# HITRainer/EAVSR

Measured on NVIDIA B200. Metric: LR frames/s, EAVSR+ x4, 270x480, higher is better.
Workload: dtype bf16

## Files before the change

### eavsr_b200/csrc/align_fused.cu

```cuda
#include "common.cuh"

namespace eavsr {
namespace {

constexpr int MX_TH = 8, MX_TW = 16;
constexpr int MX_IH = MX_TH + 4, MX_IW = MX_TW + 4;
constexpr int MX_YH = MX_TH + 2, MX_YW = MX_TW + 2;
constexpr int MX_C = 64;
constexpr int MX_THREADS = 256;

__device__ __forceinline__ void lds8(const __nv_bfloat16* p, float* f) {
  const uint4 u = *reinterpret_cast<const uint4*>(p);
  f[0] = bf16lo_to_f32(u.x); f[1] = bf16hi_to_f32(u.x); f[2] = bf16lo_to_f32(u.y); f[3] = bf16hi_to_f32(u.y);
  f[4] = bf16lo_to_f32(u.z); f[5] = bf16hi_to_f32(u.z); f[6] = bf16lo_to_f32(u.w); f[7] = bf16hi_to_f32(u.w);
}
__device__ __forceinline__ void lds8(const float* p, float* f) {
  const float4 a = *reinterpret_cast<const float4*>(p), b = *reinterpret_cast<const float4*>(p + 4);
  f[0] = a.x; f[1] = a.y; f[2] = a.z; f[3] = a.w; f[4] = b.x; f[5] = b.y; f[6] = b.z; f[7] = b.w;
}

template <typename T> struct MixSmem {
  T in[MX_IH * MX_IW][MX_C];
  T y[MX_YH * MX_YW][MX_C];
  float w1[9][MX_C];
// ... 7 lines not shown
adapt_mix_kernel(const T* __restrict__ a, const T* __restrict__ b, const T* __restrict__ w1g,
                 const T* __restrict__ b1g, const T* __restrict__ w2g, const T* __restrict__ b2g,
                 T* __restrict__ out, int H, int W, float slope) {
  extern __shared__ __align__(16) uint8_t mix_smem_raw[];
  MixSmem<T>& S = *reinterpret_cast<MixSmem<T>*>(mix_smem_raw);
  constexpr int VEC = 16 / sizeof(T);
  constexpr int CPP = MX_C / VEC;
  const int half = blockIdx.z & 1, n = blockIdx.z >> 1;
  const int y0 = blockIdx.y * MX_TH, x0 = blockIdx.x * MX_TW;
  const T* src = (half ? b : a) + (size_t)n * H * W * MX_C;
  const int tid = threadIdx.x;

  for (int i = tid; i < 9 * MX_C; i += MX_THREADS) {
    const int tap = i / MX_C, c = i % MX_C;
    S.w1[tap][c] = to_f32<T>(w1g[(size_t)(half * MX_C + c) * 9 + tap]);
    S.w2[tap][c] = to_f32<T>(w2g[((size_t)(half * (MX_C / 2) + (c >> 1)) * 2 + (c & 1)) * 9 + tap]);
  }
  for (int i = tid; i < MX_C; i += MX_THREADS) S.b1[i] = to_f32<T>(b1g[half * MX_C + i]);
  for (int i = tid; i < MX_C / 2; i += MX_THREADS) S.b2[i] = to_f32<T>(b2g[half * (MX_C / 2) + i]);

  for (int i = tid; i < MX_IH * MX_IW * CPP; i += MX_THREADS) {
    const int p = i / CPP, ch = i % CPP;
    const int gy = y0 - 2 + p / MX_IW, gx = x0 - 2 + p % MX_IW;
    const bool ok = gy >= 0 && gy < H && gx >= 0 && gx < W;
    const T* g = ok ? src + ((size_t)gy * W + gx) * MX_C + ch * VEC : src;
    const int sz = ok ? 16 : 0;
    asm volatile("cp.async.cg.shared.global [%0], [%1], 16, %2;\n" ::"r"(smem_u32(&S.in[p][ch * VEC])), "l"(g), "r"(sz));
  }
  cp_async_commit();
  cp_async_wait<0>();
  __syncthreads();

  const int c0 = (tid & 7) * 8;
  float wr[9][8], br[8];
#pragma unroll
  for (int tap = 0; tap < 9; ++tap)
#pragma unroll
    for (int e = 0; e < 8; ++e) wr[tap][e] = S.w1[tap][c0 + e];
#pragma unroll
  for (int e = 0; e < 8; ++e) br[e] = S.b1[c0 + e];

  auto st8 = [](T* p, const float* f) {
    if constexpr (sizeof(T) == 2) {
      VecLoad<T, 8>::st(p, f);
    } else {
      *reinterpret_cast<float4*>(p) = make_float4(f[0], f[1], f[2], f[3]);
      *reinterpret_cast<float4*>(p + 4) = make_float4(f[4], f[5], f[6], f[7]);
    }
  };
  static_assert(MX_YW % 2 == 0 && MX_TW % 2 == 0, "pixel pairs");
  for (int i = tid; i < MX_YH * (MX_YW / 2) * (MX_C / 8); i += MX_THREADS) {
    const int pp = i / (MX_C / 8);
    const int yy = pp / (MX_YW / 2), xx = (pp % (MX_YW / 2)) * 2;
    float acc[2][8];
#pragma unroll
    for (int e = 0; e < 8; ++e) acc[0][e] = acc[1][e] = br[e];
#pragma unroll
    for (int r = 0; r < 3; ++r) {
      float v[4][8];
#pragma unroll
      for (int c = 0; c < 4; ++c) lds8(&S.in[(yy + r) * MX_IW + xx + c][c0], v[c]);
#pragma unroll
      for (int t = 0; t < 3; ++t)
#pragma unroll
        for (int e = 0; e < 8; ++e) {
          acc[0][e] += wr[r * 3 + t][e] * v[t][e];
          acc[1][e] += wr[r * 3 + t][e] * v[t + 1][e];
        }
    }
    const int gy = y0 - 1 + yy;
#pragma unroll
    for (int k = 0; k < 2; ++k) {
      const int gx = x0 - 1 + xx + k;
      const bool inside = gy >= 0 && gy < H && gx >= 0 && gx < W;
      float o[8];
#pragma unroll
      for (int e = 0; e < 8; ++e) {
        const float v = acc[k][e] > 0.f ? acc[k][e] : acc[k][e] * slope;
        o[e] = inside ? v : 0.f;
      }
      st8(&S.y[yy * MX_YW + xx + k][c0], o);
    }
  }
  __syncthreads();

#pragma unroll
  for (int tap = 0; tap < 9; ++tap)
#pragma unroll
    for (int e = 0; e < 8; ++e) wr[tap][e] = S.w2[tap][c0 + e];
  for (int i = tid; i < MX_TH * (MX_TW / 2) * (MX_C / 8); i += MX_THREADS) {
    const int pp = i / (MX_C / 8);
    const int yy = pp / (MX_TW / 2), xx = (pp % (MX_TW / 2)) * 2;
    const int gy = y0 + yy, gx = x0 + xx;
    if (gy >= H || gx >= W) continue;
    float acc[2][4];
#pragma unroll
    for (int e = 0; e < 4; ++e) acc[0][e] = acc[1][e] = S.b2[(c0 >> 1) + e];
#pragma unroll
    for (int r = 0; r < 3; ++r) {
      float v[4][8];
#pragma unroll
      for (int c = 0; c < 4; ++c) lds8(&S.y[(yy + r) * MX_YW + xx + c][c0], v[c]);
#pragma unroll
      for (int t = 0; t < 3; ++t)
#pragma unroll
        for (int e = 0; e < 8; ++e) {
          acc[0][e >> 1] += wr[r * 3 + t][e] * v[t][e];
          acc[1][e >> 1] += wr[r * 3 + t][e] * v[t + 1][e];
        }
    }
#pragma unroll
    for (int k = 0; k < 2; ++k) {
      if (gx + k >= W) continue;
      T* op = out + ((size_t)n * H * W + (size_t)gy * W + gx + k) * MX_C + half * (MX_C / 2) + (c0 >> 1);
      float o[4];
#pragma unroll
      for (int e = 0; e < 4; ++e) o[e] = acc[k][e] > 0.f ? acc[k][e] : acc[k][e] * slope;
      if constexpr (sizeof(T) == 2) {
        *reinterpret_cast<uint2*>(op) = make_uint2(pack_bf16x2(o[0], o[1]), pack_bf16x2(o[2], o[3]));
      } else {
        *reinterpret_cast<float4*>(op) = make_float4(o[0], o[1], o[2], o[3]);
      }
    }
  }
}

template <typename T>
__global__ void __launch_bounds__(256)
affine_offsets_kernel(const T* __restrict__ tm, Strides4 ts, const T* __restrict__ tr, Strides4 rs,
                      const T* __restrict__ ml, Strides4 ms, const T* __restrict__ tm_bias,
                      const T* __restrict__ tr_bias, const T* __restrict__ ml_bias, float* __restrict__ offset,
                      float* __restrict__ mask, int N, int D, int H, int W) {
  const long long idx = (long long)blockIdx.x * blockDim.x + threadIdx.x;
  const long long HW = (long long)H * W;
  if (idx >= (long long)N * D * HW) return;
  const int pix = (int)(idx % HW);
  const int g = (int)((idx / HW) % D);
  const int n = (int)(idx / (HW * D));
  const int y = pix / W, x = pix % W;
  const T* tp = tm + n * ts.n + y * ts.h + x * ts.w + (long long)(g * 4) * ts.c;
  const T* rp = tr + n * rs.n + y * rs.h + x * rs.w + (long long)(g * 2) * rs.c;
  float a = to_f32<T>(tp[0]), b = to_f32<T>(tp[ts.c]), c = to_f32<T>(tp[2 * ts.c]), d = to_f32<T>(tp[3 * ts.c]);
  float t0 = to_f32<T>(rp[0]), t1 = to_f32<T>(rp[rs.c]);
  if (tm_bias) {
    a += to_f32<T>(tm_bias[g * 4]); b += to_f32<T>(tm_bias[g * 4 + 1]);
    c += to_f32<T>(tm_bias[g * 4 + 2]); d += to_f32<T>(tm_bias[g * 4 + 3]);
  }
  if (tr_bias) { t0 += to_f32<T>(tr_bias[g * 2]); t1 += to_f32<T>(tr_bias[g * 2 + 1]); }
  float* op = offset + ((size_t)(n * D + g) * 18) * HW + pix;
#pragma unroll
  for (int k = 0; k < 9; ++k) {
    const float r0 = (float)(k / 3 - 1), r1 = (float)(k % 3 - 1);
    op[(size_t)(2 * k) * HW] = a * r0 + b * r1 - r0 + t0;
    op[(size_t)(2 * k + 1) * HW] = c * r0 + d * r1 - r1 + t1;
  }
  if (mask) {
    const T* mp = ml + n * ms.n + y * ms.h + x * ms.w + (long long)(g * 9) * ms.c;
    float* mo = mask + ((size_t)(n * D + g) * 9) * HW + pix;
#pragma unroll
    for (int k = 0; k < 9; ++k) {
      const float lg = to_f32<T>(mp[k * ms.c]) + (ml_bias ? to_f32<T>(ml_bias[g * 9 + k]) : 0.f);
      mo[(size_t)k * HW] = 1.f / (1.f + __expf(-lg));
    }
  }
}

constexpr int CS_THREADS = 256;
constexpr int CS_PIX = 512;

template <typename T, int C, bool PROD = false>
__global__ void __launch_bounds__(CS_THREADS)
channel_sum_kernel(const T* __restrict__ x, float* __restrict__ sums, int HW, const T* __restrict__ x2 = nullptr) {
  constexpr int VEC = 16 / sizeof(T);
  constexpr int CPP = C / VEC;
  constexpr int PPI = CS_THREADS / CPP;
  __shared__ float red[PPI][C];
  const int n = blockIdx.y;
  const int ch = threadIdx.x % CPP, pl = threadIdx.x / CPP;
  const int p0 = blockIdx.x * CS_PIX;
  const int p1 = min(p0 + CS_PIX, HW);
  float acc[VEC];
#pragma unroll
  for (int e = 0; e < VEC; ++e) acc[e] = 0.f;
  const T* xn = x + (size_t)n * HW * C;
  for (int p = p0 + pl; p < p1; p += PPI) {
    float v[VEC];
    VecLoad<T, VEC>::ld(xn + (size_t)p * C + ch * VEC, v);
    if (PROD) {
      float u[VEC];
      VecLoad<T, VEC>::ld(x2 + (size_t)n * HW * C + (size_t)p * C + ch * VEC, u);
#pragma unroll
      for (int e = 0; e < VEC; ++e) acc[e] += v[e] * u[e];
    } else {
#pragma unroll
      for (int e = 0; e < VEC; ++e) acc[e] += v[e];
    }
  }
#pragma unroll
  for (int e = 0; e < VEC; ++e) red[pl][ch * VEC + e] = acc[e];
// ... 111 lines not shown
bool al16(const void* p) { return (reinterpret_cast<uintptr_t>(p) & 15u) == 0; }

template <typename T>
int mix_launch(const void* a, const void* b, const void* w1, const void* b1, const void* w2, const void* b2,
               void* out, int n, int h, int w, float slope, cudaStream_t st) {
  auto k = adapt_mix_kernel<T>;
  const int smem = (int)sizeof(MixSmem<T>);
  cudaError_t e = cudaFuncSetAttribute(k, cudaFuncAttributeMaxDynamicSharedMemorySize, smem);
  if (e != cudaSuccess) { set_error("adapt_mix: smem attr: %s", cudaGetErrorString(e)); return EAVSR_ERR_CUDA; }
  dim3 grid(ceil_div(w, MX_TW), ceil_div(h, MX_TH), n * 2);
  k<<<grid, MX_THREADS, smem, st>>>((const T*)a, (const T*)b, (const T*)w1, (const T*)b1, (const T*)w2,
                                    (const T*)b2, (T*)out, h, w, slope);
  return check_launch("adapt_mix");
}

}
}

using namespace eavsr;

extern "C" int eavsr_adapt_mix_forward(const void* a, const void* b, const void* w1, const void* b1,
                                       const void* w2, const void* b2, void* out, int n, int c, int h, int w,
                                       float negative_slope, int dtype, void* stream) {
  EAVSR_REQUIRE(a && b && w1 && b1 && w2 && b2 && out, "adapt_mix: null pointer");
  EAVSR_REQUIRE(n > 0 && h > 0 && w > 0, "adapt_mix: empty tensor");
  if (c != MX_C) { set_error("adapt_mix: only %d-channel inputs are fused (got %d)", MX_C, c); return EAVSR_ERR_UNSUPPORTED; }
  EAVSR_REQUIRE(al16(a) && al16(b) && al16(out), "adapt_mix: tensors must be 16-byte aligned dense NHWC");
  EAVSR_REQUIRE(2 * n <= 65535 && ceil_div(h, MX_TH) <= 65535, "adapt_mix: batch/height too large");
  cudaStream_t st = (cudaStream_t)stream;
  if (dtype == EAVSR_F32) return mix_launch<float>(a, b, w1, b1, w2, b2, out, n, h, w, negative_slope, st);
  if (dtype == EAVSR_BF16) return mix_launch<__nv_bfloat16>(a, b, w1, b1, w2, b2, out, n, h, w, negative_slope, st);
  set_error("adapt_mix: bad dtype %d", dtype);
  return EAVSR_ERR_INVALID;
}

extern "C" int eavsr_affine_offsets_forward(const void* transform, const int64_t transform_strides[4],
                                            const void* translation, const int64_t translation_strides[4],
                                            const void* mask_logits, const int64_t mask_strides[4],
                                            const void* transform_bias, const void* translation_bias,
                                            const void* mask_bias, float* offset, float* mask, int n,
                                            int deform_groups, int h, int w, int dtype, void* stream) {
  EAVSR_REQUIRE(transform && translation && offset && transform_strides && translation_strides,
                "affine_offsets: null pointer");
  EAVSR_REQUIRE(!mask || (mask_logits && mask_strides), "affine_offsets: mask output without logits");
  EAVSR_REQUIRE(n > 0 && deform_groups > 0 && h > 0 && w > 0, "affine_offsets: empty tensor");
  cudaStream_t st = (cudaStream_t)stream;
  Strides4 ts{transform_strides[0], transform_strides[1], transform_strides[2], transform_strides[3]};
  Strides4 rs{translation_strides[0], translation_strides[1], translation_strides[2], translation_strides[3]};
  Strides4 ms{0, 0, 0, 0};
  if (mask) ms = Strides4{mask_strides[0], mask_strides[1], mask_strides[2], mask_strides[3]};
  const long long total = (long long)n * deform_groups * h * w;
  const unsigned blocks = (unsigned)((total + 255) / 256);
  if (dtype == EAVSR_F32)
    affine_offsets_kernel<float><<<blocks, 256, 0, st>>>((const float*)transform, ts, (const float*)translation, rs,
                                                         (const float*)mask_logits, ms, (const float*)transform_bias,
                                                         (const float*)translation_bias, (const float*)mask_bias,
                                                         offset, mask, n, deform_groups, h, w);
  else if (dtype == EAVSR_BF16)
    affine_offsets_kernel<__nv_bfloat16><<<blocks, 256, 0, st>>>(
        (const __nv_bfloat16*)transform, ts, (const __nv_bfloat16*)translation, rs,
        (const __nv_bfloat16*)mask_logits, ms, (const __nv_bfloat16*)transform_bias,
        (const __nv_bfloat16*)translation_bias, (const __nv_bfloat16*)mask_bias, offset, mask, n, deform_groups, h, w);
  else { set_error("affine_offsets: bad dtype %d", dtype); return EAVSR_ERR_INVALID; }
  return check_launch("affine_offsets");
}

// ... 224 lines not shown
```

### eavsr_b200/model.py

```python
from __future__ import annotations

from collections import OrderedDict

import torch
import torch.nn as nn
import torch.nn.functional as F

from .ops import (ModulatedDeformConv2d, adapt_mix, grouped_conv3x3, grouped_conv3x3_eligible, channel_mean, scale_residual,
                  conv2d_native_bias_grad, affine_offsets_mask, ca_residual, ca_scale, cat_channels, conv2d_bias_act,
                  conv2d_bias_act_shuffle,
                  dcn_affine, dcn_affine_eligible,
                  conv3x3_64, conv3x3_64_ca, conv3x3_64_eligible, conv3x3_chain_eligible, rca_group_chain,
                  flow_warp, flow_warp2, flow_warp_nhw2, flow_warp_pyramid, flow_warp_pyramid_eligible, fused_inference_ok,
                  spynet_level_input,
                  modulated_deform_conv2d)

__all__ = ["EAVSRP", "MultiAdSTN", "SPyNet"]


class _CALayer(nn.Module):
    def __init__(self, ch=64, reduction=16):
        super().__init__()
        self.conv_du = nn.Sequential(nn.Conv2d(ch, ch // reduction, 1), nn.ReLU(inplace=True),
                                     nn.Conv2d(ch // reduction, ch, 1), nn.Sigmoid())

    def forward(self, x):
        return x * self.conv_du(channel_mean(x))


class _RCABlock(nn.Module):
    def __init__(self, ch=64):
        super().__init__()
        self.res = nn.Sequential(nn.Conv2d(ch, ch, 3, 1, 1), nn.ReLU(inplace=True), nn.Conv2d(ch, ch, 3, 1, 1))
        self.ca = _CALayer(ch)

    def forward(self, x, sums_buf=None):
        du = self.ca.conv_du
        if conv3x3_64_eligible(self.res[0], x):
            h = conv3x3_64(self.res[0], x, 0.0)
            res, sums = conv3x3_64(self.res[2], h, 1.0, want_sums=True, sums_out=sums_buf)
            return ca_scale(res, x, sums, du[0].weight, du[0].bias, du[2].weight, du[2].bias, 16)
        if x.shape[1] == 64 and fused_inference_ok(x, self.res[0].weight):
            h = conv2d_bias_act(self.res[0], x, 0.0)
            c2 = self.res[2]
            res = F.conv2d(h, c2.weight, None, c2.stride, c2.padding)
            return ca_residual(res, x, du[0].weight, du[0].bias, du[2].weight, du[2].bias, 16, res_bias=c2.bias)
# ... 75 lines not shown


def _affine_offsets(T, t, D, R=None):
    n, _, h, w = T.shape
    R = T.new_tensor(_R) if R is None else R.to(T.dtype)
    T = T.reshape(n, D, 1, 2, 2, h, w)
    Rk = R.t().reshape(1, 1, 9, 1, 2, 1, 1)
    off = (T * Rk).sum(4) - R.t().reshape(1, 1, 9, 2, 1, 1) + t.reshape(n, D, 1, 2, h, w)
    return off.reshape(n, D * 18, h, w)


class _AdaptBase(nn.Module):
    native_grouped = True

    def __init__(self, ch, n_mat, n_trans, k):
        super().__init__()
        self.register_buffer("regular_matrix", torch.tensor(_R))
        self.concat = nn.Sequential(nn.Conv2d(2 * ch, 2 * ch, 3, 1, 1, groups=2 * ch), nn.LeakyReLU(0.2, inplace=True))
        self.concat2 = nn.Sequential(nn.Conv2d(2 * ch, ch, 3, 1, 1, groups=ch), nn.LeakyReLU(0.2, inplace=True))
        self.transform_matrix_conv = nn.Conv2d(ch, n_mat, k, 1, k // 2)
        self.translation_conv = nn.Conv2d(ch, n_trans, k, 1, k // 2)

    def _merged_weight(self):
        ws = [self.transform_matrix_conv.weight, self.translation_conv.weight]
        if hasattr(self, "mask_conv"):
            ws.append(self.mask_conv.weight)
        key = tuple((w.data_ptr(), w._version, w.dtype) for w in ws)
        hit = getattr(self, "_merged", None)
        if hit is None or hit[0] != key:
            hit = (key, torch.cat([w.detach() for w in ws], 0).contiguous(memory_format=torch.channels_last))
            self._merged = hit
        return hit[1]

    def _mix(self, x, ref):
        if x.shape[1] == 64 and fused_inference_ok(x, ref):
            return adapt_mix(x, ref, self.concat[0].weight, self.concat[0].bias, self.concat2[0].weight,
                             self.concat2[0].bias, 0.2)
        xr = torch.cat([x, ref], 1)
        c1, c2 = self.concat[0], self.concat2[0]
        if self.native_grouped and grouped_conv3x3_eligible(c1, xr) and xr.dtype in (torch.float32, torch.bfloat16):
            y = F.leaky_relu(grouped_conv3x3(c1, xr), 0.2)
            if grouped_conv3x3_eligible(c2, y):
                return F.leaky_relu(grouped_conv3x3(c2, y), 0.2)
            return self.concat2(y)
        return self.concat2(self.concat(xr))


class _AdaptBlock2_3x3(_AdaptBase):

    def __init__(self, ch=64):
        super().__init__(ch, 4, 2, 3)

    def forward(self, x, ref):
        f = self._mix(x, ref)
        if fused_inference_ok(f, self.transform_matrix_conv.weight):
            ct, cr = self.transform_matrix_conv, self.translation_conv
            y = F.conv2d(f, self._merged_weight(), None, 1, ct.padding)
            return affine_offsets_mask(y[:, :4], y[:, 4:6], None, 1, ct.bias, cr.bias)[0]
        T, t = self.transform_matrix_conv(f), self.translation_conv(f)
        return _affine_offsets(T.float(), t.float(), 1, self.regular_matrix)


class _AdaptBlockOffset(_AdaptBase):

    def __init__(self, ch=64, D=8):
        super().__init__(ch, 4 * D, 2 * D, 5)
        self.D = D
        self.mask_conv = nn.Conv2d(ch, 9 * D, 5, 1, 2)

    def raw(self, x, ref):
        f = self._mix(x, ref)
        ct, cr, cm = self.transform_matrix_conv, self.translation_conv, self.mask_conv
        y = F.conv2d(f, self._merged_weight(), None, 1, ct.padding)
        key = tuple((b.data_ptr(), b._version) for b in (ct.bias, cr.bias, cm.bias))
        hit = getattr(self, "_merged_bias", None)
        if hit is None or hit[0] != key:
            hit = (key, torch.cat([ct.bias.detach(), cr.bias.detach(), cm.bias.detach()]).contiguous())
            self._merged_bias = hit
        return y, hit[1]

    def forward(self, x, ref):
        f = self._mix(x, ref)
        if fused_inference_ok(f, self.mask_conv.weight):
            ct, cr, cm = self.transform_matrix_conv, self.translation_conv, self.mask_conv
            y = F.conv2d(f, self._merged_weight(), None, 1, ct.padding)
            D = self.D
            return affine_offsets_mask(y[:, :4 * D], y[:, 4 * D:6 * D], y[:, 6 * D:], D, ct.bias, cr.bias, cm.bias)
        T, t, m = self.transform_matrix_conv(f), self.translation_conv(f), self.mask_conv(f)
        off = _affine_offsets(T.float(), t.float(), self.D, self.regular_matrix)
        return off, torch.sigmoid(m.float())


class _TransOffset(nn.Module):
    def __init__(self):
        super().__init__()
        self.conv_first = nn.Conv2d(18, 2, 3, 1, 1)

    def forward(self, off):
        return self.conv_first(off)


def _resize_flow(flow, scale):
    return F.interpolate(flow, scale_factor=scale, mode="bilinear", align_corners=True) * scale


class MultiAdSTN(ModulatedDeformConv2d):

    def __init__(self, ch=64, deformable_groups=8):
        super().__init__(ch, ch, kernel_size=3, padding=1, stride=1, dilation=1, deform_groups=deformable_groups)
        for i in (1, 2, 3):
            setattr(self, f"flow_l{i}", _AdaptBlock2_3x3(ch))
        self.adastn = _AdaptBlockOffset(ch, deformable_groups)
        self.fuse_offsets = True
        self.fold_pyramid = True
        for i in (3, 2, 1):
            setattr(self, f"trans_l{i}", _TransOffset())

    def _residual(self, lvl, warped, ref):
        off18 = getattr(self, f"flow_l{lvl}")(warped, ref)
        return getattr(self, f"trans_l{lvl}")(off18.to(warped.dtype)).float()

    def forward(self, nbr, ref, feat_prop, flow, out=None):
        flow = flow.float()
        if self.fold_pyramid and flow_warp_pyramid_eligible(nbr[0], feat_prop) and flow_warp_pyramid_eligible(nbr[1]) \
                and flow_warp_pyramid_eligible(nbr[2]) and nbr[0].dtype == torch.bfloat16:
            w3 = flow_warp_pyramid(nbr[2], [(flow, 0.25)])
            p1 = self._residual(3, w3, ref[2])
            w2, p1_up = flow_warp_pyramid(nbr[1], [(flow, 0.5), (p1, 2.0)], keep=(1,))
            p2 = self._residual(2, w2, ref[1])
            w1, flow_p2 = flow_warp_pyramid(nbr[0], [(flow, 1.0), (p2, 2.0), (p1_up, 2.0)], want_flow=True)
            p3 = self._residual(1, w1, ref[0])
            nbr_w, feat = flow_warp_pyramid(nbr[0], [(flow_p2, 1.0), (p3, 1.0)], x2=feat_prop)
            return self._deform(nbr_w, feat, ref, out)
        f4 = _resize_flow(flow, 0.25)
        f2 = _resize_flow(flow, 0.5)
        p1 = self._residual(3, flow_warp(nbr[2], f4), ref[2])
        p1_up = _resize_flow(p1, 2)
        p2 = self._residual(2, flow_warp(nbr[1], f2 + p1_up), ref[1])
        p2_up = _resize_flow(p2 + p1_up, 2)
        p3 = self._residual(1, flow_warp(nbr[0], flow + p2_up), ref[0])
        flow = p3 + p2_up + flow
        if fused_inference_ok(nbr[0], feat_prop, flow):
            nbr_w, feat = flow_warp2(nbr[0], feat_prop, flow)
        else:
            nbr_w = flow_warp(nbr[0], flow)
            feat = flow_warp(feat_prop, flow)
        return self._deform(nbr_w, feat, ref, out)

    def _deform(self, nbr_w, feat, ref, out=None):
        if (self.fuse_offsets and fused_inference_ok(nbr_w, self.adastn.mask_conv.weight)
                and nbr_w.dtype == torch.bfloat16 and tuple(self.weight.shape) == (64, 64, 3, 3)):
            y, yb = self.adastn.raw(nbr_w, ref[0])
            if dcn_affine_eligible(feat, y, self.weight, self.deform_groups):
# ... 201 lines not shown
```

### eavsr_b200/ops.py

```python
from __future__ import annotations

import math
from typing import Optional, Tuple, Union

import threading
import weakref

import ctypes

import torch
import torch.nn as nn
import torch.nn.functional as F
from torch.autograd import Function
from torch.autograd.function import once_differentiable
from torch.nn.modules.utils import _pair

from . import _lib as L

__all__ = [
    "modulated_deform_conv2d", "ModulatedDeformConv2d", "dcn_affine", "dcn_affine_eligible", "flow_warp", "flow_warp_nhw2",
    "backwarp", "get_backwarp", "invalidate_caches", "flow_warp_pyramid", "flow_warp_pyramid_eligible",
    "spynet_level_input", "cat_channels", "grouped_conv3x3", "grouped_conv3x3_eligible", "conv2d_native_bias_grad", "channel_mean", "scale_residual",
    "FunctionCorrelation", "ModuleCorrelation", "dcn_uses_tensor_cores",
    "adapt_mix", "affine_offsets_mask", "ca_residual", "fused_inference_ok", "bias_act_", "conv2d_bias_act",
    "conv3x3_64", "conv3x3_64_ca", "conv3x3_64_eligible", "ca_scale", "conv2d_bias_act_shuffle",
    "conv3x3_chain_eligible", "rca_group_chain",
]

_DTYPES = {torch.float32: L.F32, torch.bfloat16: L.BF16}


def _require_cuda(name: str, *tensors: torch.Tensor) -> None:
    for t in tensors:
        if t is not None and not t.is_cuda:
            raise NotImplementedError(
                f"eavsr_b200.{name}: CUDA tensors only (the B200 library has no CPU fallback)")


def _dtype_code(name: str, t: torch.Tensor) -> int:
    try:
        return _DTYPES[t.dtype]
    except KeyError:
        raise TypeError(f"eavsr_b200.{name}: dtype {t.dtype} not supported (float32 / bfloat16)") from None


def _strides(t: Optional[torch.Tensor]):
    if t is None:
        return None
    s = list(t.stride())
    if t.dim() == 4 and t.shape[0] == 1:
        s[0] = max(t.shape[i] * s[i] for i in (1, 2, 3))
    return L.Strides(*s)


_PLAIN_ARGS = frozenset((int, float, type(None), L.Strides))


# ... 224 lines not shown
_DCN_WS_LOCK = threading.Lock()


def _dcn_workspace(weight, dtype, ws_bytes, static):
    nothing = lambda: None
    if not static or (torch.is_grad_enabled() and weight.requires_grad):
        return torch.empty(max(ws_bytes, 16), dtype=torch.uint8, device=weight.device), False, nothing
    key = (id(weight), torch.cuda.current_stream(weight.device))
    with _DCN_WS_LOCK:
        hit = _DCN_WS_CACHE.get(key)
    if hit is not None:
        ref, version, dt, ws = hit
        if ref() is weight and version == weight._version and dt == dtype and ws.numel() >= ws_bytes \
                and ws.device == weight.device:
            return ws, True, nothing
    ws = torch.empty(max(ws_bytes, 16), dtype=torch.uint8, device=weight.device)

    def commit():
        with _DCN_WS_LOCK:
            if len(_DCN_WS_CACHE) > 256:
                for k in [k for k, v in _DCN_WS_CACHE.items() if v[0]() is None]:
                    del _DCN_WS_CACHE[k]
                if len(_DCN_WS_CACHE) > 256:
                    _DCN_WS_CACHE.clear()
            _DCN_WS_CACHE[key] = (weakref.ref(weight), weight._version, dtype, ws)
    return ws, False, commit


def invalidate_caches(module: Optional[nn.Module] = None) -> None:
    with _DCN_WS_LOCK:
        _DCN_WS_CACHE.clear()
    if module is not None:
        for m in module.modules():
            for attr in ("_eavsr_packed", "_merged", "_merged_bias"):
                if attr in m.__dict__:
                    del m.__dict__[attr]


class _ModulatedDeformConv2dFn(Function):
    @staticmethod
    def forward(ctx, input, offset, mask, weight, bias, stride, padding, dilation, groups, deform_groups,
                flags=0):
        if input is not None and input.dim() != 4:
            raise ValueError(f'Expected 4D tensor as input, got {input.dim()}D tensor instead.')
        _require_cuda("modulated_deform_conv2d", input, offset, mask, weight, bias)
        lib = L.load()
        sh, sw = _pair(stride)
        ph, pw = _pair(padding)
        dh, dw = _pair(dilation)
        cout, cin_g, kh, kw = weight.shape
        n, cin, h, w = input.shape
        ho = (h + 2 * ph - (dh * (kh - 1) + 1)) // sh + 1
        wo = (w + 2 * pw - (dw * (kw - 1) + 1)) // sw + 1
        K = kh * kw
        if cin_g * groups != cin:
            raise ValueError(f"modulated_deform_conv2d: weight {tuple(weight.shape)} does not match "
                             f"{cin} input channels with groups={groups}")
        if tuple(offset.shape) != (n, deform_groups * 2 * K, ho, wo):
            raise ValueError(f"modulated_deform_conv2d: offset shape {tuple(offset.shape)}, expected "
                             f"{(n, deform_groups * 2 * K, ho, wo)}")
        if tuple(mask.shape) != (n, deform_groups * K, ho, wo):
            raise ValueError(f"modulated_deform_conv2d: mask shape {tuple(mask.shape)}, expected "
                             f"{(n, deform_groups * K, ho, wo)}")
        code = _dtype_code("modulated_deform_conv2d", input)
        xd = _dcn_prepare_x(input, weight, groups)
        off32 = _param(offset, torch.float32)
        msk32 = _param(mask, torch.float32)
# ... 137 lines not shown
        return False
    return all(t.dtype in _DTYPES for t in ts)


def adapt_mix(a, b, w1, b1, w2, b2, negative_slope: float = 0.2):
    _require_cuda("adapt_mix", a, b, w1, b1, w2, b2)
    n, c, h, w = a.shape
    ad = a.contiguous(memory_format=torch.channels_last)
    out = torch.empty_like(ad)
    _launch("adapt_mix_forward", ad, b.to(a.dtype).contiguous(memory_format=torch.channels_last),
            *(_param(t, a.dtype) for t in (w1, b1, w2, b2)), out, n, c, h, w, float(negative_slope),
            _dtype_code("adapt_mix", ad))
    return out


def affine_offsets_mask(transform, translation, mask_logits, deform_groups: int, transform_bias=None,
                        translation_bias=None, mask_bias=None):
    _require_cuda("affine_offsets_mask", transform, translation, mask_logits)
    n, _, h, w = transform.shape
    D = deform_groups
    translation = translation.to(transform.dtype)
    offset = torch.empty((n, 18 * D, h, w), dtype=torch.float32, device=transform.device)
    mask = None
    if mask_logits is not None:
        mask_logits = mask_logits.to(transform.dtype)
        mask = torch.empty((n, 9 * D, h, w), dtype=torch.float32, device=transform.device)
    biases = [_param(t, transform.dtype) for t in (transform_bias, translation_bias, mask_bias)]
    _launch("affine_offsets_forward", transform, _strides(transform), translation, _strides(translation),
            mask_logits, _strides(mask_logits), *biases, offset, mask, n, D, h, w,
            _dtype_code("affine_offsets_mask", transform))
    return offset, mask


def dcn_affine_eligible(x, affine, weight, deform_groups: int) -> bool:
    return (deform_groups == 8 and x.dim() == 4 and x.shape[1] == 64 and x.dtype == torch.bfloat16
            and tuple(weight.shape) == (64, 64, 3, 3) and affine.dtype == torch.bfloat16
            and affine.shape[1] == 15 * deform_groups and affine.shape[0] == x.shape[0]
            and affine.shape[2:] == x.shape[2:] and x.shape[2] * x.shape[3] <= (1 << 24)
            and affine.is_contiguous(memory_format=torch.channels_last) and affine.data_ptr() % 16 == 0
            and fused_inference_ok(x, affine, weight))


def dcn_affine(x, affine, affine_bias, weight, bias, deform_groups: int = 8, static_weight: bool = False,
               flags: int = 0, out=None):
    _require_cuda("dcn_affine", x, affine, weight)
    n, c, h, w = x.shape
    xd = x.contiguous(memory_format=torch.channels_last)
    if out is None:
        out = torch.empty_like(xd)
    else:
        assert out.shape == xd.shape and out.dtype == xd.dtype and out.stride(1) == 1, "dcn_affine: bad out view"
    code = _dtype_code("dcn_affine", xd)
    ws_bytes = L.load().eavsr_dcn_forward_workspace(64, 64, 3, 3, 1, deform_groups, code)
    ws, packed, commit = _dcn_workspace(weight, x.dtype, ws_bytes, static_weight)
    if packed:
        flags |= DCN_WS_PACKED
    _launch("dcn_affine_forward", xd, _strides(xd), affine, _param(affine_bias, x.dtype), _param(weight, x.dtype),
            _param(bias, x.dtype), out, _strides(out), n, h, w, deform_groups, code, ws, ws.numel(), flags)
    commit()
    return out


def ca_residual(res, skip, w1, b1, w2, b2, reduction: int = 16, res_bias=None):
    _require_cuda("ca_residual", res, skip, w1, b1, w2, b2)
    n, c, h, w = res.shape
    rd = res.contiguous(memory_format=torch.channels_last)
# ... 327 lines not shown
```

### include/eavsr_b200.h

```cpp
#ifndef EAVSR_B200_H_
#define EAVSR_B200_H_

#include <stddef.h>
#include <stdint.h>

#ifdef __cplusplus
extern "C" {
#endif

#define EAVSR_OK 0
#define EAVSR_ERR_INVALID 1
#define EAVSR_ERR_CUDA 2
#define EAVSR_ERR_UNSUPPORTED 3

#define EAVSR_F32 0
#define EAVSR_BF16 1

#define EAVSR_FLOW_N2HW 0
#define EAVSR_FLOW_NHW2 1

#define EAVSR_PAD_ZEROS 0
#define EAVSR_PAD_BORDER 1

#define EAVSR_DCN_FORCE_GENERIC 1u
// ... 59 lines not shown
                      size_t workspace_bytes, unsigned flags, void* stream);

int eavsr_dcn_affine_forward(const void* x, const int64_t x_strides[4], const void* affine, const void* affine_bias,
                             const void* weight, const void* bias, void* out, const int64_t out_strides[4], int n,
                             int h, int w, int deform_groups, int dtype, void* workspace, size_t workspace_bytes,
                             unsigned flags, void* stream);

size_t eavsr_dcn_backward_workspace(int cin, int cout, int kh, int kw, int groups, int deform_groups, int dtype);
int eavsr_dcn_backward(const void* gout, const int64_t gout_strides[4], const void* x,
                       const int64_t x_strides[4], const float* offset, const float* mask, const void* weight,
                       float* gx32, const int64_t gx_strides[4], float* goffset, float* gmask,
                       float* gweight32, float* gbias32, int n, int cin, int h, int w, int cout, int kh, int kw,
                       int sh, int sw, int ph, int pw, int dh, int dw, int groups, int deform_groups,
                       int dtype, void* workspace, size_t workspace_bytes, unsigned flags, void* stream);

int eavsr_correlation_forward(const void* first, const void* second, void* out, int n, int c, int h, int w,
                              int dtype, void* stream);
#define EAVSR_CORR_TF32 2u
int eavsr_correlation_forward_ex(const void* first, const void* second, void* out, int n, int c, int h, int w,
                                 int dtype, unsigned flags, void* stream);
int eavsr_correlation_backward(const void* first, const void* second, const void* gout, void* gfirst,
                               void* gsecond, int n, int c, int h, int w, int dtype, void* stream);

int eavsr_adapt_mix_forward(const void* a, const void* b, const void* w1, const void* b1, const void* w2,
                            const void* b2, void* out, int n, int c, int h, int w, float negative_slope,
                            int dtype, void* stream);
int eavsr_affine_offsets_forward(const void* transform, const int64_t transform_strides[4],
                                 const void* translation, const int64_t translation_strides[4],
                                 const void* mask_logits, const int64_t mask_strides[4],
                                 const void* transform_bias ,
                                 const void* translation_bias ,
                                 const void* mask_bias , float* offset, float* mask, int n,
                                 int deform_groups, int h, int w, int dtype, void* stream);
int eavsr_ca_residual_forward(const void* res, const void* skip, const void* w1, const void* b1, const void* w2,
                              const void* b2, const void* res_bias ,
                              void* out, float* sums_workspace, int n, int c, int h, int w, int reduction, int dtype,
                              void* stream);
int eavsr_bias_act_forward(void* x, const void* bias, int c, long long pixels, float negative_slope, int dtype,
                           void* stream);

int eavsr_grouped_conv3x3_forward(const void* x, const void* weight, const void* bias, void* out, int n, int cin,
                                  int cout, int h, int w, int dtype, void* stream);
int eavsr_grouped_conv3x3_backward(const void* gout, const void* x, const void* weight, void* gx, float* gweight,
                                   float* gbias, int n, int cin, int cout, int h, int w, int dtype, void* stream);

int eavsr_channel_sum_forward(const void* x, float* sums, int n, int c, long long hw, int dtype, void* stream);

int eavsr_channel_dot_forward(const void* a, const void* b, float* sums, int n, int c, long long hw, int dtype,
                              void* stream);

int eavsr_nhwc_cat_forward(const void* const* srcs, const int* src_channels, int nsrc, void* out, int out_channels,
                           int out_channel_offset, long long pixels, int dtype, void* stream);

int eavsr_bias_act_shuffle_forward(const void* x, const void* bias, void* out, int n, int c_out, int h, int w,
                                   float negative_slope, int dtype, void* stream);
int eavsr_ca_scale_forward(const void* res, const void* skip, const float* sums, const void* w1, const void* b1,
                           const void* w2, const void* b2, const void* res_bias, void* out, int n, int c, int h,
                           int w, int reduction, int dtype, void* stream);

size_t eavsr_conv3x3_packed_weight_bytes(void);
int eavsr_conv3x3_pack_weight(const void* weight , void* packed, int cin, int cout, int dtype,
                              void* stream);
#define EAVSR_CONV_SUMS_PREZEROED 1u
int eavsr_conv3x3_forward(const void* x, const void* packed_weight, const void* bias, void* out,
                          float* channel_sums, int n, int cin, int cout, int h, int w, float negative_slope,
                          int dtype, unsigned flags, void* stream);
// ... 29 lines not shown
```

Baseline: 109.1.

## Fuse flow-head convs and affine offset expansion into one tensor-core kernel

Adds a flow_head kernel that runs the transform/translation 3x3 convs on tensor cores (ldmatrix + mma bf16). It algebraically folds the affine offset expansion and the following 18->2 conv into precomputed coefficients, so one kernel goes from mixed features straight to the 2-channel flow residual. This removes several launches and the intermediate offset tensors. The adapt_mix kernel also switches its FMA loops to paired __ffma2_rn, and the concat2 weight is cached as contiguous. The trade-off is more complex code and some precision change from the bf16 weights and the folded coefficients.

```diff
diff --git a/eavsr_b200/csrc/align_fused.cu b/eavsr_b200/csrc/align_fused.cu
--- a/eavsr_b200/csrc/align_fused.cu
+++ b/eavsr_b200/csrc/align_fused.cu
@@ -63,11 +63,12 @@
   __syncthreads();
 
   const int c0 = (tid & 7) * 8;
-  float wr[9][8], br[8];
+  float2 wr[9][4];
+  float br[8];
 #pragma unroll
   for (int tap = 0; tap < 9; ++tap)
 #pragma unroll
-    for (int e = 0; e < 8; ++e) wr[tap][e] = S.w1[tap][c0 + e];
+    for (int e = 0; e < 4; ++e) wr[tap][e] = make_float2(S.w1[tap][c0 + 2 * e], S.w1[tap][c0 + 2 * e + 1]);
 #pragma unroll
   for (int e = 0; e < 8; ++e) br[e] = S.b1[c0 + e];
 
@@ -83,9 +84,9 @@
   for (int i = tid; i < MX_YH * (MX_YW / 2) * (MX_C / 8); i += MX_THREADS) {
     const int pp = i / (MX_C / 8);
     const int yy = pp / (MX_YW / 2), xx = (pp % (MX_YW / 2)) * 2;
-    float acc[2][8];
-#pragma unroll
-    for (int e = 0; e < 8; ++e) acc[0][e] = acc[1][e] = br[e];
+    float2 acc[2][4];
+#pragma unroll
+    for (int e = 0; e < 4; ++e) acc[0][e] = acc[1][e] = make_float2(br[2 * e], br[2 * e + 1]);
 #pragma unroll
     for (int r = 0; r < 3; ++r) {
       float v[4][8];
@@ -94,9 +95,9 @@
 #pragma unroll
       for (int t = 0; t < 3; ++t)
 #pragma unroll
-        for (int e = 0; e < 8; ++e) {
-          acc[0][e] += wr[r * 3 + t][e] * v[t][e];
-          acc[1][e] += wr[r * 3 + t][e] * v[t + 1][e];
+        for (int e = 0; e < 4; ++e) {
+          acc[0][e] = __ffma2_rn(wr[r * 3 + t][e], make_float2(v[t][2 * e], v[t][2 * e + 1]), acc[0][e]);
+          acc[1][e] = __ffma2_rn(wr[r * 3 + t][e], make_float2(v[t + 1][2 * e], v[t + 1][2 * e + 1]), acc[1][e]);
         }
     }
     const int gy = y0 - 1 + yy;
@@ -107,7 +108,8 @@
       float o[8];
 #pragma unroll
       for (int e = 0; e < 8; ++e) {
-        const float v = acc[k][e] > 0.f ? acc[k][e] : acc[k][e] * slope;
+        const float a = (e & 1) ? acc[k][e >> 1].y : acc[k][e >> 1].x;
+        const float v = a > 0.f ? a : a * slope;
         o[e] = inside ? v : 0.f;
       }
       st8(&S.y[yy * MX_YW + xx + k][c0], o);
@@ -118,15 +120,19 @@
 #pragma unroll
   for (int tap = 0; tap < 9; ++tap)
 #pragma unroll
-    for (int e = 0; e < 8; ++e) wr[tap][e] = S.w2[tap][c0 + e];
+    for (int e = 0; e < 4; ++e) {
+      const int b = c0 + (e >> 1) * 4 + (e & 1);
+      wr[tap][e] = make_float2(S.w2[tap][b], S.w2[tap][b + 2]);
+    }
   for (int i = tid; i < MX_TH * (MX_TW / 2) * (MX_C / 8); i += MX_THREADS) {
     const int pp = i / (MX_C / 8);
     const int yy = pp / (MX_TW / 2), xx = (pp % (MX_TW / 2)) * 2;
     const int gy = y0 + yy, gx = x0 + xx;
     if (gy >= H || gx >= W) continue;
-    float acc[2][4];
-#pragma unroll
-    for (int e = 0; e < 4; ++e) acc[0][e] = acc[1][e] = S.b2[(c0 >> 1) + e];
+    float2 acc2[2][2];
+#pragma unroll
+    for (int q = 0; q < 2; ++q)
+      acc2[0][q] = acc2[1][q] = make_float2(S.b2[(c0 >> 1) + 2 * q], S.b2[(c0 >> 1) + 2 * q + 1]);
 #pragma unroll
     for (int r = 0; r < 3; ++r) {
       float v[4][8];
@@ -135,10 +141,16 @@
 #pragma unroll
       for (int t = 0; t < 3; ++t)
 #pragma unroll
-        for (int e = 0; e < 8; ++e) {
-          acc[0][e >> 1] += wr[r * 3 + t][e] * v[t][e];
-          acc[1][e >> 1] += wr[r * 3 + t][e] * v[t + 1][e];
+        for (int e = 0; e < 4; ++e) {
+          const int b = (e >> 1) * 4 + (e & 1);
+          acc2[0][e >> 1] = __ffma2_rn(wr[r * 3 + t][e], make_float2(v[t][b], v[t][b + 2]), acc2[0][e >> 1]);
+          acc2[1][e >> 1] = __ffma2_rn(wr[r * 3 + t][e], make_float2(v[t + 1][b], v[t + 1][b + 2]), acc2[1][e >> 1]);
         }
+    }
+    float acc[2][4];
+#pragma unroll
+    for (int k = 0; k < 2; ++k) {
+      acc[k][0] = acc2[k][0].x; acc[k][1] = acc2[k][0].y; acc[k][2] = acc2[k][1].x; acc[k][3] = acc2[k][1].y;
     }
 #pragma unroll
     for (int k = 0; k < 2; ++k) {
@@ -196,6 +208,144 @@
   }
 }
 
+constexpr int FH_TH = 16, FH_TW = 30;
+constexpr int FH_RH = FH_TH + 2, FH_RW = FH_TW + 2;
+constexpr int FH_FH = FH_TH + 4, FH_FW = FH_TW + 4;
+constexpr int FH_THREADS = 256;
+constexpr int FH_COEF = 2 * 9 * 8 + 6 + 2;
+static_assert(FH_RW == 32 && FH_RH == 18, "8 warps = 2 columns x 4 row groups (5, 5, 4, 4 rows)");
+static_assert(FH_TH % 2 == 0 && (FH_TH / 2) * FH_TW <= FH_THREADS, "stage 2: one thread per vertical pixel pair");
+
+struct FlowHeadSmem {
+  uint4 f[FH_FH * FH_FW][8];
+  float4 ya[FH_RH * FH_RW];
+  float4 yb[FH_RH * FH_RW];
+  float4 coef[FH_COEF / 4];
+};
+
+__device__ __forceinline__ void ldsm_x4(uint32_t addr, uint32_t* r) {
+  asm volatile("ldmatrix.sync.aligned.m8n8.x4.shared.b16 {%0, %1, %2, %3}, [%4];\n"
+               : "=r"(r[0]), "=r"(r[1]), "=r"(r[2]), "=r"(r[3])
+               : "r"(addr)
+               : "memory");
+}
+__device__ __forceinline__ void mma_16816(float* d, const uint32_t* a, const uint32_t* b) {
+  asm volatile("mma.sync.aligned.m16n8k16.row.col.f32.bf16.bf16.f32 {%0, %1, %2, %3}, {%4, %5, %6, %7}, {%8, %9}, "
+               "{%0, %1, %2, %3};\n"
+               : "+f"(d[0]), "+f"(d[1]), "+f"(d[2]), "+f"(d[3])
+               : "r"(a[0]), "r"(a[1]), "r"(a[2]), "r"(a[3]), "r"(b[0]), "r"(b[1]));
+}
+
+__global__ void __launch_bounds__(FH_THREADS, 2)
+flow_head_kernel(const __nv_bfloat16* __restrict__ f, const __nv_bfloat16* __restrict__ wm,
+                 const float* __restrict__ coef, float* __restrict__ p, int H, int W) {
+  extern __shared__ __align__(16) uint8_t fh_smem_raw[];
+  FlowHeadSmem& S = *reinterpret_cast<FlowHeadSmem*>(fh_smem_raw);
+  const int n = blockIdx.z, y0 = blockIdx.y * FH_TH, x0 = blockIdx.x * FH_TW;
+  const int tid = threadIdx.x, lane = tid & 31, warp = tid >> 5;
+  const __nv_bfloat16* src = f + (size_t)n * H * W * 64;
+
+  for (int i = tid; i < FH_FH * FH_FW * 8; i += FH_THREADS) {
+    const int q = i >> 3, ch = i & 7;
+    const int gy = y0 - 2 + q / FH_FW, gx = x0 - 2 + q % FH_FW;
+    const bool ok = gy >= 0 && gy < H && gx >= 0 && gx < W;
+    const __nv_bfloat16* g = ok ? src + ((size_t)gy * W + gx) * 64 + ch * 8 : src;
+    asm volatile("cp.async.cg.shared.global [%0], [%1], 16, %2;\n" ::"r"(smem_u32(&S.f[q][ch ^ (q & 7)])), "l"(g),
+                 "r"(ok ? 16 : 0));
+  }
+  cp_async_commit();
+  for (int i = tid; i < FH_COEF / 4; i += FH_THREADS) S.coef[i] = reinterpret_cast<const float4*>(coef)[i];
+
+  const int g = lane >> 2, t = lane & 3;
+  uint32_t bw[9][4][2];
+#pragma unroll
+  for (int tap = 0; tap < 9; ++tap)
+#pragma unroll
+    for (int kc = 0; kc < 4; ++kc) {
+      const uint32_t* wp = reinterpret_cast<const uint32_t*>(wm + ((g < 6 ? g : 0) * 9 + tap) * 64 + kc * 16 + 2 * t);
+      bw[tap][kc][0] = g < 6 ? __ldg(wp) : 0u;
+      bw[tap][kc][1] = g < 6 ? __ldg(wp + 4) : 0u;
+    }
+  cp_async_wait<0>();
+  __syncthreads();
+
+  const int cs = warp & 1, rg = warp >> 1;
+  const int r0 = rg * 4 + min(rg, 2), r1 = (rg + 1) * 4 + min(rg + 1, 2);
+  const uint32_t fbase = smem_u32(&S.f[0][0]);
+  const int arow = lane & 15, achunk = lane >> 4;
+  float acc[3][4];
+#pragma unroll
+  for (int d = 0; d < 3; ++d)
+#pragma unroll
+    for (int e = 0; e < 4; ++e) acc[d][e] = 0.f;
+  for (int fr = r0; fr <= r1 + 1; ++fr) {
+#pragma unroll
+    for (int dx = 0; dx < 3; ++dx) {
+      const int q = fr * FH_FW + cs * 16 + dx + arow;
+#pragma unroll
+      for (int kc = 0; kc < 4; ++kc) {
+        uint32_t a[4];
+        ldsm_x4(fbase + (uint32_t)(q * 8 + ((kc * 2 + achunk) ^ (q & 7))) * 16u, a);
+#pragma unroll
+        for (int dy = 0; dy < 3; ++dy)
+          if (fr - dy >= r0 && fr - dy < r1) mma_16816(acc[dy], a, bw[dy * 3 + dx][kc]);
+      }
+    }
+    const int rr = fr - 2;
+    if (rr >= r0) {
+      const int gy = y0 - 1 + rr;
+#pragma unroll
+      for (int hf = 0; hf < 2; ++hf) {
+        const int rc = cs * 16 + g + hf * 8, gx = x0 - 1 + rc;
+        const bool inside = gy >= 0 && gy < H && gx >= 0 && gx < W;
+        const float* bias = reinterpret_cast<const float*>(S.coef) + 144;
+        float2 v;
+        if (t < 3) v = make_float2(acc[2][2 * hf] + bias[2 * t], acc[2][2 * hf + 1] + bias[2 * t + 1]);
+        else v = make_float2(1.f, 0.f);
+        if (!inside) v = make_float2(0.f, 0.f);
+        reinterpret_cast<float2*>(t < 2 ? &S.ya[rr * FH_RW + rc] : &S.yb[rr * FH_RW + rc])[t & 1] = v;
+      }
+    }
+#pragma unroll
+    for (int e = 0; e < 4; ++e) {
+      acc[2][e] = acc[1][e];
+      acc[1][e] = acc[0][e];
+      acc[0][e] = 0.f;
+    }
+  }
+  __syncthreads();
+
+  const size_t plane = (size_t)H * W;
+  const int oy = (tid / FH_TW) * 2, ox = tid % FH_TW, gy = y0 + oy, gx = x0 + ox;
+  if (tid < (FH_TH / 2) * FH_TW && gy < H && gx < W) {
+    const float4 bo = S.coef[FH_COEF / 4 - 1];
+    float s[2][2] = {{bo.z, bo.w}, {bo.z, bo.w}};
+#pragma unroll
+    for (int r = 0; r < 4; ++r)
+#pragma unroll
+      for (int kx = 0; kx < 3; ++kx) {
+        const float4 u = S.ya[(oy + r) * FH_RW + ox + kx], v = S.yb[(oy + r) * FH_RW + ox + kx];
+#pragma unroll
+        for (int k = 0; k < 2; ++k) {
+          if (r - k < 0 || r - k > 2) continue;
+          const int j = (r - k) * 3 + kx;
+#pragma unroll
+          for (int o = 0; o < 2; ++o) {
+            const float4 c = S.coef[(o * 9 + j) * 2], d = S.coef[(o * 9 + j) * 2 + 1];
+            s[k][o] += c.x * u.x + c.y * u.y + c.z * u.z + c.w * u.w + d.x * v.x + d.y * v.y + d.z * v.z;
+          }
+        }
+      }
+    float* op = p + (size_t)n * 2 * plane + (size_t)gy * W + gx;
+    op[0] = s[0][0];
+    op[plane] = s[0][1];
+    if (gy + 1 < H) {
+      op[W] = s[1][0];
+      op[plane + W] = s[1][1];
+    }
+  }
+}
+
 constexpr int CS_THREADS = 256;
 constexpr int CS_PIX = 512;
 
@@ -373,6 +523,24 @@
   if (dtype == EAVSR_BF16) return mix_launch<__nv_bfloat16>(a, b, w1, b1, w2, b2, out, n, h, w, negative_slope, st);
   set_error("adapt_mix: bad dtype %d", dtype);
   return EAVSR_ERR_INVALID;
+}
+
+extern "C" int eavsr_flow_head_forward(const void* f, const void* merged_weight, const float* coef, float* out, int n,
+                                       int c, int h, int w, void* stream) {
+  EAVSR_REQUIRE(f && merged_weight && coef && out, "flow_head: null pointer");
+  EAVSR_REQUIRE(n > 0 && h > 0 && w > 0, "flow_head: empty tensor");
+  if (c != 64) { set_error("flow_head: only 64-channel inputs are fused (got %d)", c); return EAVSR_ERR_UNSUPPORTED; }
+  EAVSR_REQUIRE(al16(f), "flow_head: f must be a 16-byte aligned dense NHWC tensor");
+  EAVSR_REQUIRE((reinterpret_cast<uintptr_t>(merged_weight) & 3u) == 0, "flow_head: merged_weight must be 4-byte aligned");
+  EAVSR_REQUIRE(n <= 65535 && ceil_div(h, FH_TH) <= 65535, "flow_head: batch/height too large");
+  auto k = flow_head_kernel;
+  const int smem = (int)sizeof(FlowHeadSmem);
+  cudaError_t e = cudaFuncSetAttribute(k, cudaFuncAttributeMaxDynamicSharedMemorySize, smem);
+  if (e != cudaSuccess) { set_error("flow_head: smem attr: %s", cudaGetErrorString(e)); return EAVSR_ERR_CUDA; }
+  dim3 grid(ceil_div(w, FH_TW), ceil_div(h, FH_TH), n);
+  k<<<grid, FH_THREADS, smem, (cudaStream_t)stream>>>((const __nv_bfloat16*)f, (const __nv_bfloat16*)merged_weight, coef,
+                                                      out, h, w);
+  return check_launch("flow_head");
 }
 
 extern "C" int eavsr_affine_offsets_forward(const void* transform, const int64_t transform_strides[4],
diff --git a/eavsr_b200/model.py b/eavsr_b200/model.py
--- a/eavsr_b200/model.py
+++ b/eavsr_b200/model.py
@@ -12,6 +12,7 @@
                   dcn_affine, dcn_affine_eligible,
                   conv3x3_64, conv3x3_64_ca, conv3x3_64_eligible, conv3x3_chain_eligible, rca_group_chain,
                   flow_warp, flow_warp2, flow_warp_nhw2, flow_warp_pyramid, flow_warp_pyramid_eligible, fused_inference_ok,
+                  flow_head, flow_head_eligible, flow_head_weights,
                   spynet_level_input,
                   modulated_deform_conv2d)
 
@@ -153,9 +154,18 @@
             self._merged = hit
         return hit[1]
 
+    def _concat2_weight(self):
+        w = self.concat2[0].weight
+        key = (w.data_ptr(), w._version, w.dtype)
+        hit = getattr(self, "_concat2_w", None)
+        if hit is None or hit[0] != key:
+            hit = (key, w.detach().contiguous())
+            self._concat2_w = hit
+        return hit[1]
+
     def _mix(self, x, ref):
         if x.shape[1] == 64 and fused_inference_ok(x, ref):
-            return adapt_mix(x, ref, self.concat[0].weight, self.concat[0].bias, self.concat2[0].weight,
+            return adapt_mix(x, ref, self.concat[0].weight, self.concat[0].bias, self._concat2_weight(),
                              self.concat2[0].bias, 0.2)
         xr = torch.cat([x, ref], 1)
         c1, c2 = self.concat[0], self.concat2[0]
@@ -173,7 +183,9 @@
         super().__init__(ch, 4, 2, 3)
 
     def forward(self, x, ref):
-        f = self._mix(x, ref)
+        return self.offsets(self._mix(x, ref))
+
+    def offsets(self, f):
         if fused_inference_ok(f, self.transform_matrix_conv.weight):
             ct, cr = self.transform_matrix_conv, self.translation_conv
             y = F.conv2d(f, self._merged_weight(), None, 1, ct.padding)
@@ -234,12 +246,23 @@
         self.adastn = _AdaptBlockOffset(ch, deformable_groups)
         self.fuse_offsets = True
         self.fold_pyramid = True
+        self.fuse_flow_head = True
         for i in (3, 2, 1):
             setattr(self, f"trans_l{i}", _TransOffset())
 
     def _residual(self, lvl, warped, ref):
-        off18 = getattr(self, f"flow_l{lvl}")(warped, ref)
-        return getattr(self, f"trans_l{lvl}")(off18.to(warped.dtype)).float()
+        blk, trans = getattr(self, f"flow_l{lvl}"), getattr(self, f"trans_l{lvl}")
+        f = blk._mix(warped, ref)
+        ct, cr, c2 = blk.transform_matrix_conv, blk.translation_conv, trans.conv_first
+        if self.fuse_flow_head and flow_head_eligible(f, ct.weight, cr.weight, c2.weight):
+            params = (ct.weight, ct.bias, cr.weight, cr.bias, c2.weight, c2.bias)
+            key = tuple((t.data_ptr(), t._version) for t in params)
+            hit = getattr(trans, "_flow_head", None)
+            if hit is None or hit[0] != key:
+                hit = (key, flow_head_weights(*params))
+                trans._flow_head = hit
+            return flow_head(f, hit[1])
+        return trans(blk.offsets(f).to(warped.dtype)).float()
 
     def forward(self, nbr, ref, feat_prop, flow, out=None):
         flow = flow.float()
diff --git a/eavsr_b200/ops.py b/eavsr_b200/ops.py
--- a/eavsr_b200/ops.py
+++ b/eavsr_b200/ops.py
@@ -22,7 +22,7 @@
     "backwarp", "get_backwarp", "invalidate_caches", "flow_warp_pyramid", "flow_warp_pyramid_eligible",
     "spynet_level_input", "cat_channels", "grouped_conv3x3", "grouped_conv3x3_eligible", "conv2d_native_bias_grad", "channel_mean", "scale_residual",
     "FunctionCorrelation", "ModuleCorrelation", "dcn_uses_tensor_cores",
-    "adapt_mix", "affine_offsets_mask", "ca_residual", "fused_inference_ok", "bias_act_", "conv2d_bias_act",
+    "adapt_mix", "affine_offsets_mask", "flow_head", "flow_head_eligible", "flow_head_weights", "ca_residual", "fused_inference_ok", "bias_act_", "conv2d_bias_act",
     "conv3x3_64", "conv3x3_64_ca", "conv3x3_64_eligible", "ca_scale", "conv2d_bias_act_shuffle",
     "conv3x3_chain_eligible", "rca_group_chain",
 ]
@@ -313,7 +313,7 @@
         _DCN_WS_CACHE.clear()
     if module is not None:
         for m in module.modules():
-            for attr in ("_eavsr_packed", "_merged", "_merged_bias"):
+            for attr in ("_eavsr_packed", "_merged", "_merged_bias", "_concat2_w", "_flow_head"):
                 if attr in m.__dict__:
                     del m.__dict__[attr]
 
@@ -517,6 +517,38 @@
     return offset, mask
 
 
+def flow_head_eligible(f, transform_weight, translation_weight, trans_weight) -> bool:
+    return (f.dim() == 4 and f.shape[1] == 64 and f.dtype == torch.bfloat16
+            and f.is_contiguous(memory_format=torch.channels_last) and f.data_ptr() % 16 == 0
+            and tuple(transform_weight.shape) == (4, 64, 3, 3) and tuple(translation_weight.shape) == (2, 64, 3, 3)
+            and tuple(trans_weight.shape) == (2, 18, 3, 3)
+            and fused_inference_ok(f, transform_weight, translation_weight, trans_weight))
+
+
+def flow_head_weights(transform_weight, transform_bias, translation_weight, translation_bias, trans_weight,
+                      trans_bias):
+    wm = torch.cat([transform_weight.detach(), translation_weight.detach()], 0).to(torch.bfloat16)
+    wm = wm.permute(0, 2, 3, 1).contiguous()
+    w = trans_weight.detach().double().reshape(2, 9, 2, 9)
+    k = torch.arange(9, device=w.device, dtype=torch.float64)
+    r0, r1 = (torch.div(k, 3, rounding_mode="floor") - 1)[:, None], (k % 3 - 1)[:, None]
+    we, wo = w[:, :, 0], w[:, :, 1]
+    g = torch.stack([(we * r0).sum(1), (we * r1).sum(1), (wo * r0).sum(1), (wo * r1).sum(1), we.sum(1), wo.sum(1),
+                     -(we * r0 + wo * r1).sum(1), torch.zeros_like(we[:, 0])], -1)
+    coef = torch.cat([g.reshape(-1), transform_bias.detach().double(), translation_bias.detach().double(),
+                      trans_bias.detach().double()]).float()
+    return wm, coef
+
+
+def flow_head(f, weights):
+    _require_cuda("flow_head", f)
+    n, c, h, w = f.shape
+    wm, coef = weights
+    out = torch.empty((n, 2, h, w), dtype=torch.float32, device=f.device)
+    _launch("flow_head_forward", f, wm, coef, out, n, c, h, w)
+    return out
+
+
 def dcn_affine_eligible(x, affine, weight, deform_groups: int) -> bool:
     return (deform_groups == 8 and x.dim() == 4 and x.shape[1] == 64 and x.dtype == torch.bfloat16
             and tuple(weight.shape) == (64, 64, 3, 3) and affine.dtype == torch.bfloat16
diff --git a/include/eavsr_b200.h b/include/eavsr_b200.h
--- a/include/eavsr_b200.h
+++ b/include/eavsr_b200.h
@@ -115,6 +115,8 @@
                                  const void* translation_bias ,
                                  const void* mask_bias , float* offset, float* mask, int n,
                                  int deform_groups, int h, int w, int dtype, void* stream);
+int eavsr_flow_head_forward(const void* f, const void* merged_weight, const float* coef, float* out, int n, int c,
+                            int h, int w, void* stream);
 int eavsr_ca_residual_forward(const void* res, const void* skip, const void* w1, const void* b1, const void* w2,
                               const void* b2, const void* res_bias ,
                               void* out, float* sums_workspace, int n, int c, int h, int w, int reduction, int dtype,
```

Result: faster. 112.6, median of 6 (+3.2%).
